# MP-Gadget/MP-Gadget

Measured on AMD Instinct MI355X. Metric: particle-updates/sec (gravity force step: PM + tree build + short-range walk), higher is better.
Workload: dtype f64; 1 GPU; 256^3 DM-only TreePM force step, Nmesh=512, s_zel ICs, all particles active, relative opening criterion (ErrTolForceAcc 0.002), TreeRcut 6, Asmth 1.5; particles=16777216, nmesh=512, parallelism=1 GPU

## Files before the change

### mp-gadget_amd/csrc/pm.h

```cpp
#pragma once
#include "../../include/mpgadget_hip.h"
#include "mpg_common.h"
#include "tree_build.h"
#include <rocfft/rocfft.h>
#include <cmath>
#include <vector>

namespace mpg {

struct FftPlan {
    rocfft_plan plan = nullptr;
    rocfft_execution_info info = nullptr;
    DevBuf<char> work;
    void create(rocfft_result_placement placement, rocfft_transform_type type, int dims, const size_t *lengths, size_t batch);
    void exec(void *in, void *out, hipStream_t st);
    void destroy();
    bool ready() const { return plan != nullptr; }
};

struct PMesh {
    double box = 0, Asmth = 0, G = 0, cellsize = 0;
    int nmesh = 0;
    bool have_plans = false;
    bool kspace_force = false;
    FftPlan plan_r2c, plan_c2r;
    DevBuf<double> real;
    DevBuf<double> rho_k;
    DevBuf<double> work_k;
    DevBuf<double> invsinc2, difffac;
    struct DepositState {
        int mode = 0, since_tune = 0;
    } dep_single, dep_slab;
    void deposit(int64_t n, const double *d_pos, const float *d_mass, const uint8_t *d_active, double *mesh, int x0, int P, DepositState &ds,
                 hipStream_t st, EventTimer *tm);
    DevBuf<unsigned long long> dep_keys_a, dep_keys_b;
    DevBuf<int> dep_idx_a, dep_idx_b;
    DevBuf<char> dep_tmp;
    bool measure_power = true, ps_valid = false;
    int ps_nmesh = 0;
    DevBuf<double> ps_acc;
    DevBuf<unsigned long long> ps_modes;
    void ps_zero(hipStream_t st);
    double asmth2() const { return pow((2 * M_PI) * Asmth / nmesh, 2); }
    double pot_factor() const { return -G / (M_PI * box); }
    enum { TR_MEASURE = 1, TR_APPLY = 2, TR_BOTH = 3 };
    template <bool XLAST, bool FUSE, bool NU> void measure_spectrum(double *rho, int ny, int y0, unsigned grid, hipStream_t st);
    template <bool XLAST, bool FUSE> void transfer_stage(int parts, double *rho, int ny, int y0, unsigned grid, hipStream_t st);
    size_t ps_lds_bytes() const { return (size_t)nmesh * 3 * sizeof(double); }

    mpg_nu_response_fn nu_fn = nullptr;
    void *nu_ctx = nullptr;
    double nu_box_mpc = 0;
    int nu_nonzero = 0;
    const char *nu_who = "gravpm_force";
    double nu_prefac = 0, nu_normfac = 1;
    DevBuf<double> nu_tab;
    DevBuf<int> nu_guess;
    double *nu_host = nullptr;
    size_t nu_host_cap = 0;
    size_t ps_lds_bytes_nu() const { return ps_lds_bytes() + (size_t)nmesh * (2 * sizeof(double) + sizeof(int)); }
    void nu_fetch(hipStream_t st, double **acc, unsigned long long **modes);
    void nu_table(const double *acc, const unsigned long long *modes, hipStream_t st);
    DepositState dep_plane;
    DevBuf<double> ps_keep;
    double plane_nu_correction(int64_t n, const double *d_pos, const float *d_mass, const uint8_t *d_active, mpg_nu_response_fn fn, void *ctx,
                               double box_mpc, hipStream_t st);
    bool hybrid_tracer = false;
    DevBuf<float> tracer_mass_buf;
    const float *tracer_mass(int64_t n, const float *d_mass, const uint8_t *d_type, hipStream_t st);

    void init(double BoxSize, double Asmth, int Nmesh, double G, hipStream_t st);
    void ensure_single();
    void destroy();
    void force(int64_t n, const double *d_pos, const float *d_mass, const uint8_t *d_active, double *d_gravpm, double *d_potential,
               hipStream_t st, EventTimer *tm);
    ~PMesh() { destroy(); }

    struct Slab {
// ... 26 lines not shown
```

### mp-gadget_amd/csrc/pm.hip

```cpp
#include "pm.h"
#include "pm_cic.h"
#include <algorithm>
#include <cmath>
#include <cstdlib>
#include <cstring>
#include <rocprim/rocprim.hpp>

namespace mpg {

#define MPG_FFT(expr)                                                                                          \
    do {                                                                                                       \
        rocfft_status _r = (expr);                                                                             \
        if(_r != rocfft_status_success)                                                                        \
            ::mpg::fail(__FILE__, __LINE__, std::string("rocFFT error ") + std::to_string((int)_r) + " in " #expr); \
    } while(0)

__global__ void __launch_bounds__(256) k_cic_deposit(int64_t n, const double *__restrict__ pos, const float *__restrict__ mass,
                                                     const uint8_t *__restrict__ active, double cellsize, int nmesh,
                                                     double *__restrict__ mesh)
{
    const int64_t i = (int64_t)blockIdx.x * blockDim.x + threadIdx.x;
    if(i >= n)
        return;
    if(active && !active[i])
        return;
    int ic[3];
    double res[3];
    cic_cell3(pos + 3 * i, cellsize, nmesh, ic, res);
    const double m = (double)mass[i];
#pragma unroll
    for(int c = 0; c < 8; c++)
        unsafeAtomicAdd(&mesh[cic_index(c, ic, nmesh)], cic_weight(c, res, 1.0) * m);
}

__global__ void __launch_bounds__(256) k_cic_deposit_slab(int64_t n, const double *__restrict__ pos, const float *__restrict__ mass,
                                                          const uint8_t *__restrict__ active, double cellsize, int nmesh, int x0, int P,
                                                          double *__restrict__ slab)
{
    const int64_t i = (int64_t)blockIdx.x * blockDim.x + threadIdx.x;
    if(i >= n)
        return;
    if(active && !active[i])
        return;
    int ic[3];
    double res[3];
    ic[0] = cic_cell(pos[3 * i], cellsize, nmesh, res[0]);
    if(!in_slab(ic[0], x0, P) && !in_slab(wrap(ic[0] + 1, nmesh), x0, P))
        return;
#pragma unroll
    for(int k = 1; k < 3; k++)
        ic[k] = cic_cell(pos[3 * i + k], cellsize, nmesh, res[k]);
    const double m = (double)mass[i];
#pragma unroll
    for(int c = 0; c < 8; c++) {
        size_t lin;
        if(cic_index_slab(c, ic, nmesh, x0, P, lin))
            unsafeAtomicAdd(&slab[lin], cic_weight(c, res, 1.0) * m);
    }
}

__global__ void __launch_bounds__(256) k_cell_keys(int64_t n, const double *__restrict__ pos, const uint8_t *__restrict__ active, double cellsize,
                                                   int nmesh, unsigned long long *__restrict__ keys, int *__restrict__ idx)
{
    const int64_t i = (int64_t)blockIdx.x * blockDim.x + threadIdx.x;
    if(i >= n)
        return;
    int ic[3];
    double res[3];
    cic_cell3(pos + 3 * i, cellsize, nmesh, ic, res);
    keys[i] = (active && !active[i]) ? ~0ull : (unsigned long long)cic_index(0, ic, nmesh);
    idx[i] = (int)i;
}

__global__ void __launch_bounds__(256) k_cic_deposit_sorted(int64_t n, const unsigned long long *__restrict__ skeys, const int *__restrict__ sidx,
                                                            const double *__restrict__ pos, const float *__restrict__ mass, double cellsize,
                                                            int nmesh, int x0, int P, double *__restrict__ mesh)
{
    const int64_t k = (int64_t)blockIdx.x * blockDim.x + threadIdx.x;
    const int lane = threadIdx.x & 63;
    unsigned long long key = ~0ull;
    double w[8];
    int ic[3] = {0, 0, 0};
#pragma unroll
    for(int c = 0; c < 8; c++)
        w[c] = 0;
    if(k < n) {
        key = skeys[k];
        if(key != ~0ull) {
            const int i = sidx[k];
            double res[3];
            cic_cell3(pos + 3 * (int64_t)i, cellsize, nmesh, ic, res);
            const double m = (double)mass[i];
#pragma unroll
            for(int c = 0; c < 8; c++)
                w[c] = cic_weight(c, res, m);
        }
    }
    const unsigned long long prev = __shfl_up(key, 1);
    bool f = lane == 0 || prev != key;
    const bool head_next = __shfl_down(f ? 1 : 0, 1) != 0;
    const bool tail = lane == 63 || head_next;
    for(int d = 1; d < 64; d <<= 1) {
        const bool f2 = __shfl_up(f ? 1 : 0, d) != 0;
        double v2[8];
#pragma unroll
        for(int c = 0; c < 8; c++)
            v2[c] = __shfl_up(w[c], d);
        if(lane >= d && !f) {
#pragma unroll
            for(int c = 0; c < 8; c++)
                w[c] += v2[c];
            f = f2;
        }
    }
    if(tail && key != ~0ull) {
#pragma unroll
        for(int c = 0; c < 8; c++) {
            size_t lin;
            if(cic_index_slab(c, ic, nmesh, x0, P, lin))
                unsafeAtomicAdd(&mesh[lin], w[c]);
        }
    }
}

__device__ __forceinline__ double sinc_unnormed(double x)
{
    if(x < 1e-5 && x > -1e-5) {
        const double x2 = x * x;
        return 1.0 - x2 / 6. + x2 * x2 / 120.;
    }
    return sin(x) / x;
}

struct FourierCell {
    int ix, iy, iz;
    long long k2;
};
template <bool XLAST>
__device__ __forceinline__ FourierCell fourier_cell(size_t ip, int nmesh, int ny, int y0)
{
    const int nz = nmesh / 2 + 1;
    FourierCell c;
    if(XLAST) {
        c.ix = (int)(ip % nmesh);
        const size_t j = ip / nmesh;
        c.iz = (int)(j % nz);
        c.iy = y0 + (int)(j / nz);
    }
    else {
        c.iz = (int)(ip % nz);
        const size_t t = ip / nz;
        c.iy = y0 + (int)(t % ny);
        c.ix = (int)(t / ny);
    }
    const int kx = c.ix <= nmesh / 2 ? c.ix : c.ix - nmesh;
    const int ky = c.iy <= nmesh / 2 ? c.iy : c.iy - nmesh;
    const int kz = c.iz;
    c.k2 = (long long)kx * kx + (long long)ky * ky + (long long)kz * kz;
    return c;
}

__device__ __forceinline__ double potential_fac(long long k2, double asmth2, double pot_factor, double f)
{
    const double smth = exp(-(double)k2 * asmth2) / (double)k2;
    return pot_factor * smth * f * f;
}

__device__ __forceinline__ int logk_bin(long long k2, double binsperunit) { return (int)floor(binsperunit * log((double)k2) / 2.); }

template <bool XLAST>
__global__ void __launch_bounds__(256) k_potential_transfer(int nmesh, int ny, int y0, double asmth2, double pot_factor,
                                                            const double *__restrict__ invsinc2, double2 *__restrict__ cplx)
{
    const int nz = nmesh / 2 + 1;
    const size_t total = (size_t)nmesh * ny * nz;
    const size_t ip = (size_t)blockIdx.x * blockDim.x + threadIdx.x;
    if(ip >= total)
        return;
    const FourierCell c = fourier_cell<XLAST>(ip, nmesh, ny, y0);
    double2 v = cplx[ip];
    if(c.k2 == 0) {
        v.x = 0.0;
        v.y = 0.0;
    }
    else {
        const double fac = potential_fac(c.k2, asmth2, pot_factor, invsinc2[c.ix] * invsinc2[c.iy] * invsinc2[c.iz]);
        v.x *= fac;
        v.y *= fac;
    }
    cplx[ip] = v;
}

struct NuArgs {
    const double *tab;
    const int *guess;
    int nonzero;
    double prefac, normfac;
    double kscale;
};

__device__ __forceinline__ double nu_factor(double x, int kint, const double *s_lk, const double *s_rt, const int *s_gs, int nonzero,
                                            double prefac)
{
    const double x0 = s_lk[0], x1 = s_lk[nonzero - 1];
    if(x < x0 && x > x0 - log(2.0))
        x = x0;
    else if(x > x1)
        x = x1;
    x = x < x0 ? x0 : x;
    int j = s_gs[kint];
    while(j > 0 && x < s_lk[j])
        j--;
    while(j < nonzero - 2 && x >= s_lk[j + 1])
        j++;
    const double x_lo = s_lk[j], x_hi = s_lk[j + 1], y_lo = s_rt[j], y_hi = s_rt[j + 1];
    return 1 + prefac * (y_lo + (x - x_lo) / (x_hi - x_lo) * (y_hi - y_lo));
}

template <bool XLAST, bool FUSE = false, bool NU = false>
__global__ void __launch_bounds__(256) k_power_spectrum(int nmesh, int ny, int y0, const double *__restrict__ invsinc2,
                                                        double2 *__restrict__ cplx, double *__restrict__ acc,
                                                        unsigned long long *__restrict__ modes, double asmth2 = 0, double pot_factor = 0,
                                                        NuArgs nu = NuArgs{})
{
    extern __shared__ double s_ps[];
    const int nbins = nmesh;
    double *s_pow = s_ps, *s_kk = s_ps + nbins;
    unsigned long long *s_n = (unsigned long long *)(s_ps + 2 * nbins);
    double *s_lk = s_ps + 3 * nbins, *s_rt = s_ps + 4 * nbins;
    int *s_gs = (int *)(s_ps + 5 * nbins);
    for(int b = threadIdx.x; b < nbins; b += blockDim.x) {
        s_pow[b] = 0;
        s_kk[b] = 0;
        s_n[b] = 0;
        if(NU) {
            s_lk[b] = nu.tab[b];
            s_rt[b] = nu.tab[nbins + b];
            s_gs[b] = nu.guess[b];
        }
    }
    __syncthreads();
    const int nz = nmesh / 2 + 1;
    const size_t total = (size_t)nmesh * ny * nz;
    const double binsperunit = (nbins - 1) / log(sqrt(3.0) * nmesh / 2.0);
    for(size_t ip = (size_t)blockIdx.x * blockDim.x + threadIdx.x; ip < total; ip += (size_t)gridDim.x * blockDim.x) {
        const FourierCell fc = fourier_cell<XLAST>(ip, nmesh, ny, y0);
        const long long k2 = fc.k2;
        double2 v = cplx[ip];
        if(k2 == 0) {
            const double m0 = v.x * v.x + v.y * v.y;
            acc[2 * nbins] = NU ? m0 * nu.normfac : m0;
            if(FUSE)
                cplx[ip] = make_double2(0.0, 0.0);
            continue;
        }
        int kint = 0;
        if(NU) {
            kint = logk_bin(k2, binsperunit);
            const double nufac = nu_factor(log(sqrt((double)k2) * nu.kscale), kint < nbins ? kint : nbins - 1, s_lk, s_rt, s_gs, nu.nonzero,
                                           nu.prefac);
            v.x *= nufac;
            v.y *= nufac;
            if(!FUSE)
                cplx[ip] = v;
        }
        const double m = v.x * v.x + v.y * v.y;
        const double f = invsinc2[fc.ix] * invsinc2[fc.iy] * invsinc2[fc.iz];
        if(FUSE) {
            const double fac = potential_fac(k2, asmth2, pot_factor, f);
            cplx[ip] = make_double2(v.x * fac, v.y * fac);
        }
        if(!NU)
            kint = logk_bin(k2, binsperunit);
        if(kint >= nbins)
            continue;
        const int w = (fc.iz == 0 || fc.iz == nmesh / 2) ? 1 : 2;
        __hip_atomic_fetch_add(&s_pow[kint], w * m * f * f, __ATOMIC_RELAXED, __HIP_MEMORY_SCOPE_WORKGROUP);
        __hip_atomic_fetch_add(&s_kk[kint], w * sqrt((double)k2), __ATOMIC_RELAXED, __HIP_MEMORY_SCOPE_WORKGROUP);
        __hip_atomic_fetch_add(&s_n[kint], (unsigned long long)w, __ATOMIC_RELAXED, __HIP_MEMORY_SCOPE_WORKGROUP);
    }
    __syncthreads();
    for(int b = threadIdx.x; b < nbins; b += blockDim.x)
        if(s_n[b]) {
            unsafeAtomicAdd(&acc[b], s_pow[b]);
            unsafeAtomicAdd(&acc[nbins + b], s_kk[b]);
            atomicAdd(&modes[b], s_n[b]);
        }
}

__global__ void __launch_bounds__(256) k_nu_correction(int nmesh, double2 *__restrict__ cplx, NuArgs nu)
{
    extern __shared__ double s_ps[];
    const int nbins = nmesh;
    double *s_lk = s_ps, *s_rt = s_ps + nbins;
    int *s_gs = (int *)(s_ps + 2 * nbins);
    for(int b = threadIdx.x; b < nbins; b += blockDim.x) {
        s_lk[b] = nu.tab[b];
        s_rt[b] = nu.tab[nbins + b];
        s_gs[b] = nu.guess[b];
    }
    __syncthreads();
    const int nz = nmesh / 2 + 1;
    const size_t total = (size_t)nmesh * nmesh * nz;
    const double binsperunit = (nbins - 1) / log(sqrt(3.0) * nmesh / 2.0);
    for(size_t ip = (size_t)blockIdx.x * blockDim.x + threadIdx.x; ip < total; ip += (size_t)gridDim.x * blockDim.x) {
        const long long k2 = fourier_cell<false>(ip, nmesh, nmesh, 0).k2;
        if(k2 == 0) {
            cplx[ip] = make_double2(0.0, 0.0);
            continue;
        }
        const int kint = logk_bin(k2, binsperunit);
        const double f = nu_factor(log(sqrt((double)k2) * nu.kscale), kint < nbins ? kint : nbins - 1, s_lk, s_rt, s_gs, nu.nonzero, nu.prefac) - 1;
        double2 v = cplx[ip];
        v.x *= f;
        v.y *= f;
        cplx[ip] = v;
    }
}

template <bool XLAST>
__global__ void __launch_bounds__(256) k_force_transfer(int nmesh, int ny, int y0, int axis, const double *__restrict__ difffac,
                                                        const double2 *__restrict__ src, double2 *__restrict__ dst, int xmul, int xoff)
{
    const int nz = nmesh / 2 + 1;
    const size_t total = (size_t)nmesh * ny * nz;
    const size_t ip = (size_t)blockIdx.x * blockDim.x + threadIdx.x;
    if(ip >= total)
        return;
    double2 v = src[ip];
    const FourierCell fc = fourier_cell<XLAST>(ip, nmesh, ny, y0);
    if(axis >= 0) {
        const double fac = difffac[axis == 0 ? fc.ix : (axis == 1 ? fc.iy : fc.iz)];
        const double t0 = -v.y * fac, t1 = v.x * fac;
        v.x = t0;
        v.y = t1;
    }
    const size_t rowsz = (size_t)ny * nz;
    if(XLAST)
        dst[ip] = v;
    else
// ... 96 lines not shown
        is2[i] = 1. / (s * s);
        const double w = k * (2 * M_PI / nmesh);
        dff[i] = -1 * (1 / 6.0 * (8 * sin(w) - sin(2 * w))) * (nmesh / box);
    }
    invsinc2.reserve(nmesh);
    difffac.reserve(nmesh);
    MPG_HIP(hipMemcpyAsync(invsinc2.p, is2.data(), nmesh * sizeof(double), hipMemcpyHostToDevice, st));
    MPG_HIP(hipMemcpyAsync(difffac.p, dff.data(), nmesh * sizeof(double), hipMemcpyHostToDevice, st));
    MPG_HIP(hipStreamSynchronize(st));
}

void FftPlan::create(rocfft_result_placement placement, rocfft_transform_type type, int dims, const size_t *lengths, size_t batch)
{
    static const bool once = (rocfft_setup(), true);
    (void)once;
    destroy();
    MPG_FFT(rocfft_plan_create(&plan, placement, type, rocfft_precision_double, (size_t)dims, lengths, batch, nullptr));
    MPG_FFT(rocfft_execution_info_create(&info));
    size_t wb = 0;
    MPG_FFT(rocfft_plan_get_work_buffer_size(plan, &wb));
    if(wb > 0) {
        work.reserve(wb + 64);
        MPG_FFT(rocfft_execution_info_set_work_buffer(info, work.p, wb));
    }
}

void FftPlan::exec(void *in, void *out, hipStream_t st)
{
    MPG_FFT(rocfft_execution_info_set_stream(info, st));
    void *ib[1] = {in}, *ob[1] = {out};
    MPG_FFT(rocfft_execute(plan, ib, out == in ? nullptr : ob, info));
}

void FftPlan::destroy()
{
    if(info)
        (void)rocfft_execution_info_destroy(info);
    if(plan)
        (void)rocfft_plan_destroy(plan);
    info = nullptr;
    plan = nullptr;
    work.release();
}

void PMesh::ensure_single()
{
    if(have_plans)
        return;
    const size_t nreal = (size_t)nmesh * nmesh * nmesh;
    const size_t ncplx = (size_t)nmesh * nmesh * (nmesh / 2 + 1);
    real.reserve(nreal);
    rho_k.reserve(2 * ncplx);
    work_k.reserve(2 * ncplx);
    const size_t len3[3] = {(size_t)nmesh, (size_t)nmesh, (size_t)nmesh};
    plan_r2c.create(rocfft_placement_notinplace, rocfft_transform_type_real_forward, 3, len3, 1);
    plan_c2r.create(rocfft_placement_notinplace, rocfft_transform_type_real_inverse, 3, len3, 1);
    have_plans = true;
}

void PMesh::ps_zero(hipStream_t st)
{
    ps_acc.reserve(2 * (size_t)nmesh + 8);
    ps_modes.reserve((size_t)nmesh + 8);
    MPG_HIP(hipMemsetAsync(ps_acc.p, 0, (2 * (size_t)nmesh + 1) * sizeof(double), st));
    MPG_HIP(hipMemsetAsync(ps_modes.p, 0, (size_t)nmesh * sizeof(unsigned long long), st));
    ps_valid = true;
    ps_nmesh = nmesh;
}

void PMesh::nu_fetch(hipStream_t st, double **acc, unsigned long long **modes)
{
    const size_t nb = (size_t)nmesh, want = 3 * nb + 1;
    if(nu_host_cap < want) {
        if(nu_host)
            (void)hipHostFree(nu_host);
        nu_host = nullptr;
        nu_host_cap = 0;
        MPG_HIP(hipHostMalloc((void **)&nu_host, want * sizeof(double), hipHostMallocDefault));
        nu_host_cap = want;
    }
    MPG_HIP(hipMemcpyAsync(nu_host, ps_acc.p, (2 * nb + 1) * sizeof(double), hipMemcpyDeviceToHost, st));
    MPG_HIP(hipMemcpyAsync(nu_host + 2 * nb + 1, ps_modes.p, nb * sizeof(unsigned long long), hipMemcpyDeviceToHost, st));
    MPG_HIP(hipStreamSynchronize(st));
    *acc = nu_host;
    *modes = (unsigned long long *)(nu_host + 2 * nb + 1);
}

void PMesh::nu_table(const double *acc, const unsigned long long *modes, hipStream_t st)
{
    const int nb = nmesh;
    MPG_CHECK(ps_lds_bytes_nu() <= 65536, std::string(nu_who) + ": the neutrino response keeps its table in LDS: Nmesh " + std::to_string(nmesh) + " is too large");
    std::vector<double> kk(nb), dcdm(nb), tab(2 * (size_t)nb, 0.0);
    std::vector<int64_t> nm(nb);
    int nonzero = 0;
    if(mpg_powerspectrum_sum(nb, acc, (const int64_t *)modes, nu_box_mpc, kk.data(), dcdm.data(), nm.data(), &nonzero) != 0)
        throw Error(mpg_last_error());
    for(int i = 0; i < nonzero; i++)
        dcdm[i] = sqrt(dcdm[i]);
    double prefac = NAN, mtot = NAN;
    double *lk = tab.data(), *rt = tab.data() + nb;
    for(int i = 0; i < nonzero; i++)
        lk[i] = rt[i] = NAN;
    const int rc = nu_fn(nu_ctx, nonzero, kk.data(), dcdm.data(), nm.data(), lk, rt, &prefac, &mtot);
    MPG_CHECK(rc == 0, std::string(nu_who) + ": the neutrino response callback failed (returned " + std::to_string(rc) + ")");
    MPG_CHECK(nonzero >= 2, std::string(nu_who) + ": neutrino response table: " + std::to_string(nonzero) + " power spectrum bins, at least 2 needed");
    MPG_CHECK(std::isfinite(prefac) && std::isfinite(mtot), std::string(nu_who) + ": neutrino response callback: nu_prefac / MtotbyMcdm not finite");
    for(int i = 0; i < nonzero; i++) {
        MPG_CHECK(std::isfinite(lk[i]) && std::isfinite(rt[i]),
                  std::string(nu_who) + ": neutrino response table: entry " + std::to_string(i) + " is not finite");
        MPG_CHECK(i == 0 || lk[i] > lk[i - 1], std::string(nu_who) + ": neutrino response table: logknu is not strictly increasing at entry " + std::to_string(i));
    }
    std::vector<int> guess(nb);
    int c = 0;
    for(int b = 0; b < nb; b++) {
        guess[b] = std::min(std::max(c - 1, 0), nonzero - 2);
        if(modes[b])
            c++;
    }
    nu_tab.reserve(2 * (size_t)nb);
    nu_guess.reserve((size_t)nb);
    memcpy(nu_host, tab.data(), 2 * (size_t)nb * sizeof(double));
    memcpy(nu_host + 2 * (size_t)nb, guess.data(), (size_t)nb * sizeof(int));
    MPG_HIP(hipMemcpyAsync(nu_tab.p, nu_host, 2 * (size_t)nb * sizeof(double), hipMemcpyHostToDevice, st));
    MPG_HIP(hipMemcpyAsync(nu_guess.p, nu_host + 2 * (size_t)nb, (size_t)nb * sizeof(int), hipMemcpyHostToDevice, st));
    nu_nonzero = nonzero;
    nu_prefac = prefac;
    nu_normfac = mtot * mtot;
    ps_zero(st);
}

__global__ void __launch_bounds__(256) k_tracer_mass(int64_t n, const float *__restrict__ mass, const uint8_t *__restrict__ type,
                                                     float *__restrict__ out)
{
    const int64_t i = (int64_t)blockIdx.x * blockDim.x + threadIdx.x;
    if(i < n)
        out[i] = type[i] == 2 ? 0.0f : mass[i];
}

const float *PMesh::tracer_mass(int64_t n, const float *d_mass, const uint8_t *d_type, hipStream_t st)
{
    if(!hybrid_tracer || n <= 0)
        return d_mass;
    MPG_CHECK(d_type != nullptr, "gravpm_force: the hybrid-neutrino deposit mask needs the particle types");
    tracer_mass_buf.reserve((size_t)n);
    hipLaunchKernelGGL(k_tracer_mass, dim3(nblk(n)), dim3(256), 0, st, n, d_mass, d_type, tracer_mass_buf.p);
    return tracer_mass_buf.p;
}

void PMesh::destroy()
{
    if(have_plans) {
        plan_r2c.destroy();
        plan_c2r.destroy();
        have_plans = false;
    }
    slab_destroy();
    real.release();
    rho_k.release();
    work_k.release();
    if(nu_host)
        (void)hipHostFree(nu_host);
    nu_host = nullptr;
    nu_host_cap = 0;
    nmesh = 0;
}

void PMesh::deposit(int64_t n, const double *d_pos, const float *d_mass, const uint8_t *d_active, double *mesh, int x0, int P, DepositState &ds,
                    hipStream_t st, EventTimer *tm)
{
    const size_t ncell = (size_t)P * nmesh * nmesh, nreal = (size_t)nmesh * nmesh * nmesh;
    const bool whole = x0 == 0 && P == nmesh;
    auto plain = [&]() {
        if(whole)
            hipLaunchKernelGGL(k_cic_deposit, dim3(nblk(n)), dim3(256), 0, st, n, d_pos, d_mass, d_active, cellsize, nmesh, mesh);
        else
            hipLaunchKernelGGL(k_cic_deposit_slab, dim3(nblk(n)), dim3(256), 0, st, n, d_pos, d_mass, d_active, cellsize, nmesh, x0, P, mesh);
    };
    auto sorted = [&]() {
        dep_keys_a.reserve((size_t)n + 1);
        dep_keys_b.reserve((size_t)n + 1);
        dep_idx_a.reserve((size_t)n + 1);
        dep_idx_b.reserve((size_t)n + 1);
        hipLaunchKernelGGL(k_cell_keys, dim3(nblk(n)), dim3(256), 0, st, n, d_pos, d_active, cellsize, nmesh, dep_keys_a.p, dep_idx_a.p);
        int bits = 1;
        while(bits < 64 && ((unsigned long long)1 << bits) < (unsigned long long)nreal)
            bits++;
        size_t tb = 0;
        MPG_HIP(rocprim::radix_sort_pairs(nullptr, tb, dep_keys_a.p, dep_keys_b.p, dep_idx_a.p, dep_idx_b.p, (size_t)n, 0, 64, st));
        dep_tmp.reserve(tb + 16);
        MPG_HIP(rocprim::radix_sort_pairs((void *)dep_tmp.p, tb, dep_keys_a.p, dep_keys_b.p, dep_idx_a.p, dep_idx_b.p, (size_t)n, 0,
                                          d_active ? 64 : bits, st));
        hipLaunchKernelGGL(k_cic_deposit_sorted, dim3(nblk(n)), dim3(256), 0, st, n, dep_keys_b.p, dep_idx_b.p, d_pos, d_mass, cellsize, nmesh, x0, P,
                           mesh);
    };
    if(const char *e = getenv("MPG_PM_DEPOSIT"))
        ds.mode = !strcmp(e, "sorted") ? 2 : 1;
    if(ds.mode == 0 || ++ds.since_tune >= 64) {
        hipEvent_t e0, e1, e2;
        MPG_HIP(hipEventCreate(&e0));
        MPG_HIP(hipEventCreate(&e1));
        MPG_HIP(hipEventCreate(&e2));
        MPG_HIP(hipEventRecord(e0, st));
        sorted();
        MPG_HIP(hipEventRecord(e1, st));
        MPG_HIP(hipMemsetAsync(mesh, 0, ncell * sizeof(double), st));
        plain();
        MPG_HIP(hipEventRecord(e2, st));
        MPG_HIP(hipEventSynchronize(e2));
        float ts = 0, tp = 0;
        MPG_HIP(hipEventElapsedTime(&ts, e0, e1));
        MPG_HIP(hipEventElapsedTime(&tp, e1, e2));
        (void)hipEventDestroy(e0);
        (void)hipEventDestroy(e1);
        (void)hipEventDestroy(e2);
        ds.mode = ts < tp ? 2 : 1;
        ds.since_tune = 0;
        if(tm)
            tm->start(st);
        MPG_HIP(hipMemsetAsync(mesh, 0, ncell * sizeof(double), st));
    }
    if(ds.mode == 2)
        sorted();
    else
        plain();
}

template <bool XLAST, bool FUSE, bool NU>
void PMesh::measure_spectrum(double *rho, int ny, int y0, unsigned grid, hipStream_t st)
{
    if(!NU)
        ps_zero(st);
    const NuArgs na = NU ? NuArgs{nu_tab.p, nu_guess.p, nu_nonzero, nu_prefac, nu_normfac, 2 * M_PI / nu_box_mpc} : NuArgs{};
    hipLaunchKernelGGL((k_power_spectrum<XLAST, FUSE, NU>), dim3(grid), dim3(256), NU ? ps_lds_bytes_nu() : ps_lds_bytes(), st, nmesh, ny, y0,
                       invsinc2.p, (double2 *)rho, ps_acc.p, ps_modes.p, FUSE ? asmth2() : 0.0, FUSE ? pot_factor() : 0.0, na);
}

template <bool XLAST, bool FUSE>
void PMesh::transfer_stage(int parts, double *rho, int ny, int y0, unsigned grid, hipStream_t st)
{
    if((parts & TR_MEASURE) && (nu_fn || (measure_power && !FUSE)))
        measure_spectrum<XLAST, false, false>(rho, ny, y0, grid, st);
    if(parts == TR_BOTH && nu_fn) {
        double *acc;
        unsigned long long *modes;
        nu_fetch(st, &acc, &modes);
        nu_table(acc, modes, st);
    }
    if(!(parts & TR_APPLY))
        return;
    if(nu_fn)
        measure_spectrum<XLAST, FUSE, true>(rho, ny, y0, grid, st);
    else if(FUSE && measure_power)
        measure_spectrum<XLAST, FUSE, false>(rho, ny, y0, grid, st);
    if(!FUSE || !(nu_fn || measure_power))
        hipLaunchKernelGGL(k_potential_transfer<XLAST>, dim3(nblk((size_t)nmesh * ny * (nmesh / 2 + 1))), dim3(256), 0, st, nmesh, ny, y0, asmth2(),
                           pot_factor(), invsinc2.p, (double2 *)rho);
}

double PMesh::plane_nu_correction(int64_t n, const double *d_pos, const float *d_mass, const uint8_t *d_active, mpg_nu_response_fn fn, void *ctx,
                                  double box_mpc, hipStream_t st)
{
    MPG_CHECK(nmesh > 0, "potential planes: the massive-neutrino correction needs the PM mesh (gravpm_init_periodic first)");
    MPG_CHECK(!slab.ready, "potential planes: the massive-neutrino correction is not available while the mesh is in its slab-decomposed form");
    MPG_CHECK(fn && box_mpc > 0, "potential planes: the massive-neutrino correction needs a callback and BoxSize_in_MPC > 0");
    ensure_single();
    const size_t nreal = (size_t)nmesh * nmesh * nmesh, nb = (size_t)nmesh;
    const bool had_ps = ps_valid && ps_nmesh == nmesh;
    if(had_ps) {
        ps_keep.reserve(3 * nb + 1);
        MPG_HIP(hipMemcpyAsync(ps_keep.p, ps_acc.p, (2 * nb + 1) * sizeof(double), hipMemcpyDeviceToDevice, st));
        MPG_HIP(hipMemcpyAsync(ps_keep.p + 2 * nb + 1, ps_modes.p, nb * sizeof(unsigned long long), hipMemcpyDeviceToDevice, st));
    }
    struct Restore {
        PMesh *pm;
        mpg_nu_response_fn fn;
        void *ctx;
        double box_mpc, prefac, normfac;
        int nonzero;
        bool had_ps;
        hipStream_t st;
        ~Restore()
        {
            pm->nu_who = "gravpm_force";
            pm->nu_fn = fn;
            pm->nu_ctx = ctx;
            pm->nu_box_mpc = box_mpc;
            pm->nu_prefac = prefac;
            pm->nu_normfac = normfac;
            pm->nu_nonzero = nonzero;
            pm->ps_valid = had_ps;
            if(had_ps) {
                const size_t nb = (size_t)pm->nmesh;
                (void)hipMemcpyAsync(pm->ps_acc.p, pm->ps_keep.p, (2 * nb + 1) * sizeof(double), hipMemcpyDeviceToDevice, st);
                (void)hipMemcpyAsync(pm->ps_modes.p, pm->ps_keep.p + 2 * nb + 1, nb * sizeof(unsigned long long), hipMemcpyDeviceToDevice, st);
            }
        }
    } restore{this, nu_fn, nu_ctx, nu_box_mpc, nu_prefac, nu_normfac, nu_nonzero, had_ps, st};
    MPG_HIP(hipMemsetAsync(real.p, 0, nreal * sizeof(double), st));
    if(n > 0)
        deposit(n, d_pos, d_mass, d_active, real.p, 0, nmesh, dep_plane, st, nullptr);
    plan_r2c.exec(real.p, rho_k.p, st);
    measure_spectrum<false, false, false>(rho_k.p, nmesh, 0, 2048, st);
    double total_mass = 0;
    MPG_HIP(hipMemcpyAsync(&total_mass, rho_k.p, sizeof(double), hipMemcpyDeviceToHost, st));
    double *acc;
    unsigned long long *modes;
    nu_fetch(st, &acc, &modes);
    MPG_CHECK(total_mass > 0, "potential planes: cannot build a potential plane from zero active particle mass");
    nu_who = "potential planes";
    nu_fn = fn;
    nu_ctx = ctx;
    nu_box_mpc = box_mpc;
    nu_table(acc, modes, st);
    const NuArgs na{nu_tab.p, nu_guess.p, nu_nonzero, nu_prefac, nu_normfac, 2 * M_PI / nu_box_mpc};
    hipLaunchKernelGGL(k_nu_correction, dim3(2048), dim3(256), (size_t)nmesh * (2 * sizeof(double) + sizeof(int)), st, nmesh, (double2 *)rho_k.p, na);
    MPG_HIP(hipGetLastError());
    plan_c2r.exec(rho_k.p, real.p, st);
    return total_mass;
}

void PMesh::force(int64_t n, const double *d_pos, const float *d_mass, const uint8_t *d_active, double *d_gravpm, double *d_potential,
                  hipStream_t st, EventTimer *tm)
{
    MPG_CHECK(nmesh > 0, "gravpm_force called before gravpm_init_periodic");
    MPG_CHECK(!slab.ready, "gravpm_force: the mesh is in its slab-decomposed form (use the pm_slab calls)");
    ensure_single();
    const size_t nreal = (size_t)nmesh * nmesh * nmesh;
    const size_t ncplx = (size_t)nmesh * nmesh * (nmesh / 2 + 1);
    float t_fft = 0, t_tr = 0, t_ro = 0;
    auto lap = [&](float &sum) {
        float t;
        if(tm) {
            tm->lap(st, &t);
            sum += t;
        }
    };
    if(tm)
        tm->start(st);
    MPG_HIP(hipMemsetAsync(real.p, 0, nreal * sizeof(double), st));
    if(n > 0)
        deposit(n, d_pos, d_mass, d_active, real.p, 0, nmesh, dep_single, st, tm);
    if(tm)
        tm->lap(st, &tm->t.pm_deposit);
    plan_r2c.exec(real.p, rho_k.p, st);
    lap(t_fft);
    static const bool fuse_ps = !(getenv("MPG_PM_FUSE_PS") && getenv("MPG_PM_FUSE_PS")[0] == '0');
    if(fuse_ps)
        transfer_stage<false, true>(TR_BOTH, rho_k.p, nmesh, 0, 2048, st);
    else
        transfer_stage<false, false>(TR_BOTH, rho_k.p, nmesh, 0, 2048, st);
    lap(t_tr);
    if(!kspace_force) {
        plan_c2r.exec(rho_k.p, real.p, st);
        lap(t_fft);
        if(n > 0)
            hipLaunchKernelGGL(k_cic_readout_stencil, dim3(nblk(n)), dim3(256), 0, st, n, d_pos, d_active, cellsize, nmesh, (double)nmesh / box,
                               (const double *)real.p, d_gravpm, d_potential);
        lap(t_ro);
    }
    else
        for(int f = 0; f < 4; f++) {
        const int axis = f - 1;
        if(f == 0 && !d_potential)
            continue;
        hipLaunchKernelGGL(k_force_transfer<false>, dim3(nblk(ncplx)), dim3(256), 0, st, nmesh, nmesh, 0, axis, difffac.p,
                           (const double2 *)rho_k.p, (double2 *)work_k.p, 1, 0);
        lap(t_tr);
        plan_c2r.exec(work_k.p, real.p, st);
        lap(t_fft);
        if(n > 0) {
            if(f == 0)
                hipLaunchKernelGGL(k_cic_readout, dim3(nblk(n)), dim3(256), 0, st, n, d_pos, d_active, cellsize, nmesh, real.p, 3, d_potential);
            else
                hipLaunchKernelGGL(k_cic_readout, dim3(nblk(n)), dim3(256), 0, st, n, d_pos, d_active, cellsize, nmesh, real.p, axis, d_gravpm);
        }
        lap(t_ro);
    }
    MPG_HIP(hipGetLastError());
    if(tm && tm->enabled) {
        tm->t.pm_fft = t_fft;
        tm->t.pm_transfer = t_tr;
        tm->t.pm_readout = t_ro;
        tm->t.pm_total = tm->t.pm_deposit + t_fft + t_tr + t_ro;
    }
}


__global__ void __launch_bounds__(256) k_slab_pack_a(int nmesh, int P, int Py, const double2 *__restrict__ C, double2 *__restrict__ sendA)
{
    const int nz = nmesh / 2 + 1;
    const size_t total = (size_t)P * nmesh * nz;
    const size_t ip = (size_t)blockIdx.x * blockDim.x + threadIdx.x;
    if(ip >= total)
        return;
    const int iz = (int)(ip % nz);
    const size_t t = ip / nz;
    const int y = (int)(t % nmesh);
    const int xl = (int)(t / nmesh);
    const int d = y / Py, yl = y - d * Py;
    sendA[(((size_t)d * P + xl) * Py + yl) * nz + iz] = C[ip];
}

__global__ void __launch_bounds__(256) k_slab_unpack_b(int nmesh, int P, int Py, const double2 *__restrict__ recvB, double2 *__restrict__ C)
{
    const int nz = nmesh / 2 + 1;
    const size_t total = (size_t)P * nmesh * nz;
// ... 11 lines not shown
__global__ void __launch_bounds__(256) k_transpose(int rows, int cols, const double2 *__restrict__ in, size_t in_ld, double2 *__restrict__ out,
                                                   size_t out_ld)
{
    __shared__ double2 tile[32][33];
    const int tx = threadIdx.x & 31, ty = threadIdx.x >> 5;
    const int c0 = blockIdx.x * 32, r0 = blockIdx.y * 32;
#pragma unroll
    for(int k = 0; k < 32; k += 8) {
        const int r = r0 + ty + k, c = c0 + tx;
        if(r < rows && c < cols)
            tile[ty + k][tx] = in[(size_t)r * in_ld + c];
    }
    __syncthreads();
#pragma unroll
    for(int k = 0; k < 32; k += 8) {
        const int c = c0 + ty + k, r = r0 + tx;
        if(r < rows && c < cols)
            out[(size_t)c * out_ld + r] = tile[tx][ty + k];
    }
}

void PMesh::slab_destroy()
{
    if(slab.ready) {
        slab.p2d_r2c.destroy();
        slab.p2d_c2r.destroy();
        slab.p1d_fwd.destroy();
        slab.p1d_inv.destroy();
        slab.ready = false;
    }
    slab.phi.release();
    slab.force.release();
    slab.C.release();
    slab.rho_k.release();
    slab.work.release();
}

void PMesh::slab_init(int rank, int world)
{
    MPG_CHECK(nmesh > 0, "pm_slab_init called before gravpm_init_periodic");
    MPG_CHECK(world >= 1 && rank >= 0 && rank < world, "pm_slab_init: bad rank / world");
    MPG_CHECK(nmesh % world == 0, "pm_slab_init: Nmesh must be a multiple of the number of GPUs");
    slab_destroy();
    slab.rank = rank;
    slab.world = world;
    slab.P = slab.Py = nmesh / world;
    const int nz = nmesh / 2 + 1;
    const size_t S = (size_t)slab.Py * nz;
    MPG_CHECK(slab.P >= 3, "pm_slab_init: at least 3 mesh planes per GPU are needed");
    slab.phi.reserve((size_t)(slab.P + 5) * nmesh * nmesh);
    slab.force.reserve((size_t)(slab.P + 1) * nmesh * nmesh);
    slab.C.reserve(2 * (size_t)slab.P * nmesh * nz);
    slab.rho_k.reserve(2 * (size_t)nmesh * S);
    if(have_plans) {
        plan_r2c.destroy();
        plan_c2r.destroy();
        have_plans = false;
    }
    real.release();
    rho_k.release();
    work_k.release();
    const size_t len2[2] = {(size_t)nmesh, (size_t)nmesh}, len1[1] = {(size_t)nmesh};
    slab.p2d_r2c.create(rocfft_placement_notinplace, rocfft_transform_type_real_forward, 2, len2, (size_t)slab.P);
    slab.p2d_c2r.create(rocfft_placement_notinplace, rocfft_transform_type_real_inverse, 2, len2, (size_t)slab.P);
    slab.p1d_fwd.create(rocfft_placement_inplace, rocfft_transform_type_complex_forward, 1, len1, S);
    slab.p1d_inv.create(rocfft_placement_inplace, rocfft_transform_type_complex_inverse, 1, len1, S);
    slab.work.reserve(2 * (size_t)nmesh * S);
    slab.ready = true;
}

void PMesh::slab_forward_a(int64_t n, const double *d_pos, const float *d_mass, double *sendA, hipStream_t st)
{
    MPG_CHECK(slab.ready, "pm_slab: not initialised");
    const int nz = nmesh / 2 + 1;
    const size_t nreal = (size_t)slab.P * nmesh * nmesh;
    MPG_HIP(hipMemsetAsync(slab.force.p, 0, nreal * sizeof(double), st));
    if(n > 0)
        deposit(n, d_pos, d_mass, nullptr, slab.force.p, slab.rank * slab.P, slab.P, dep_slab, st, nullptr);
    slab.p2d_r2c.exec(slab.force.p, slab.C.p, st);
    hipLaunchKernelGGL(k_slab_pack_a, dim3(nblk((size_t)slab.P * nmesh * nz)), dim3(256), 0, st, nmesh, slab.P, slab.Py, (const double2 *)slab.C.p,
                       (double2 *)sendA);
    MPG_HIP(hipGetLastError());
}

void PMesh::slab_forward_b(double *recvA, double *sendB, hipStream_t st)
{
    slab_forward_b1(recvA, st);
    slab_forward_b2(sendB, st);
}

void PMesh::slab_forward_b1(double *recvA, hipStream_t st)
{
    MPG_CHECK(slab.ready, "pm_slab: not initialised");
    const int nz = nmesh / 2 + 1;
    const int y0 = slab.rank * slab.Py;
    const size_t S = (size_t)slab.Py * nz;
    const dim3 tgrid_f((unsigned)((S + 31) / 32), (unsigned)((nmesh + 31) / 32));
    hipLaunchKernelGGL(k_transpose, tgrid_f, dim3(256), 0, st, nmesh, (int)S, (const double2 *)recvA, S, (double2 *)slab.rho_k.p, (size_t)nmesh);
    slab.p1d_fwd.exec(slab.rho_k.p, slab.rho_k.p, st);
    transfer_stage<true, false>(TR_MEASURE, slab.rho_k.p, slab.Py, y0, 1024, st);
}

void PMesh::slab_forward_b2(double *sendB, hipStream_t st)
{
    MPG_CHECK(slab.ready, "pm_slab: not initialised");
    const int nz = nmesh / 2 + 1;
    const int y0 = slab.rank * slab.Py;
    const size_t S = (size_t)slab.Py * nz;
    const dim3 tgrid_b((unsigned)((nmesh + 31) / 32), (unsigned)((S + 31) / 32));
    transfer_stage<true, false>(TR_APPLY, slab.rho_k.p, slab.Py, y0, 1024, st);
    slab.p1d_inv.exec(slab.rho_k.p, slab.rho_k.p, st);
// ... 55 lines not shown
```

Measured before the change: 237.4 million particles/s.

## Fuse x-axis FFT passes with PM transfer and spectrum into one kernel

Replaces the full 3D r2c/c2r rocFFT plans with batched 2D plans over the y/z axes plus a custom kernel that performs the x-axis forward FFT, applies the potential transfer function and power-spectrum binning, then runs the inverse x-axis FFT in LDS. This removes two full passes over the complex mesh, since the transfer stage and the x-direction FFT passes no longer each stream the mesh through global memory. Separately, CIC deposit now uses two threads per particle, each handling four of the eight corners. The hand-written radix-8/4/2 FFT trades rocFFT's tuning for custom code, with possible register and LDS pressure and numerical-accuracy risk.

```diff
diff --git a/mp-gadget_amd/csrc/pm.h b/mp-gadget_amd/csrc/pm.h
--- a/mp-gadget_amd/csrc/pm.h
+++ b/mp-gadget_amd/csrc/pm.h
@@ -24,6 +24,13 @@
     bool have_plans = false;
     bool kspace_force = false;
     FftPlan plan_r2c, plan_c2r;
+    FftPlan plan2_r2c, plan2_c2r;
+    DevBuf<double> xp_tw;
+    int xp_blocks = 0;
+    bool xpass_usable() const;
+    void ensure_3d();
+    void ensure_xpass(hipStream_t st);
+    void xpass_solve(hipStream_t st);
     DevBuf<double> real;
     DevBuf<double> rho_k;
     DevBuf<double> work_k;
diff --git a/mp-gadget_amd/csrc/pm.hip b/mp-gadget_amd/csrc/pm.hip
--- a/mp-gadget_amd/csrc/pm.hip
+++ b/mp-gadget_amd/csrc/pm.hip
@@ -19,7 +19,9 @@
                                                      const uint8_t *__restrict__ active, double cellsize, int nmesh,
                                                      double *__restrict__ mesh)
 {
-    const int64_t i = (int64_t)blockIdx.x * blockDim.x + threadIdx.x;
+    const int64_t t = (int64_t)blockIdx.x * blockDim.x + threadIdx.x;
+    const int64_t i = t >> 1;
+    const int h = (int)(t & 1);
     if(i >= n)
         return;
     if(active && !active[i])
@@ -29,8 +31,10 @@
     cic_cell3(pos + 3 * i, cellsize, nmesh, ic, res);
     const double m = (double)mass[i];
 #pragma unroll
-    for(int c = 0; c < 8; c++)
+    for(int q = 0; q < 4; q++) {
+        const int c = 4 * h + q;
         unsafeAtomicAdd(&mesh[cic_index(c, ic, nmesh)], cic_weight(c, res, 1.0) * m);
+    }
 }
 
 __global__ void __launch_bounds__(256) k_cic_deposit_slab(int64_t n, const double *__restrict__ pos, const float *__restrict__ mass,
@@ -136,6 +140,13 @@
     int ix, iy, iz;
     long long k2;
 };
+__device__ __forceinline__ long long fourier_k2(int ix, int iy, int iz, int nmesh)
+{
+    const int kx = ix <= nmesh / 2 ? ix : ix - nmesh;
+    const int ky = iy <= nmesh / 2 ? iy : iy - nmesh;
+    const int kz = iz;
+    return (long long)kx * kx + (long long)ky * ky + (long long)kz * kz;
+}
 template <bool XLAST>
 __device__ __forceinline__ FourierCell fourier_cell(size_t ip, int nmesh, int ny, int y0)
 {
@@ -153,10 +164,7 @@
         c.iy = y0 + (int)(t % ny);
         c.ix = (int)(t / ny);
     }
-    const int kx = c.ix <= nmesh / 2 ? c.ix : c.ix - nmesh;
-    const int ky = c.iy <= nmesh / 2 ? c.iy : c.iy - nmesh;
-    const int kz = c.iz;
-    c.k2 = (long long)kx * kx + (long long)ky * ky + (long long)kz * kz;
+    c.k2 = fourier_k2(c.ix, c.iy, c.iz, nmesh);
     return c;
 }
 
@@ -215,6 +223,62 @@
         j++;
     const double x_lo = s_lk[j], x_hi = s_lk[j + 1], y_lo = s_rt[j], y_hi = s_rt[j + 1];
     return 1 + prefac * (y_lo + (x - x_lo) / (x_hi - x_lo) * (y_hi - y_lo));
+}
+
+struct PsLds {
+    double *pow, *kk;
+    unsigned long long *n;
+    const double *lk, *rt;
+    const int *gs;
+};
+
+__device__ __forceinline__ double ps_binsperunit(int nmesh) { return (nmesh - 1) / log(sqrt(3.0) * nmesh / 2.0); }
+
+template <bool FUSE, bool NU>
+__device__ __forceinline__ bool spectrum_mode(const FourierCell &fc, int nmesh, double binsperunit, const double *__restrict__ invsinc2, double2 &v,
+                                              const PsLds &s, double *__restrict__ acc, double asmth2, double pot_factor, const NuArgs &nu)
+{
+    const int nbins = nmesh;
+    const long long k2 = fc.k2;
+    if(k2 == 0) {
+        const double m0 = v.x * v.x + v.y * v.y;
+        acc[2 * nbins] = NU ? m0 * nu.normfac : m0;
+        if(FUSE)
+            v = make_double2(0.0, 0.0);
+        return FUSE;
+    }
+    int kint = 0;
+    if(NU) {
+        kint = logk_bin(k2, binsperunit);
+        const double nufac = nu_factor(log(sqrt((double)k2) * nu.kscale), kint < nbins ? kint : nbins - 1, s.lk, s.rt, s.gs, nu.nonzero, nu.prefac);
+        v.x *= nufac;
+        v.y *= nufac;
+    }
+    const double m = v.x * v.x + v.y * v.y;
+    const double f = invsinc2[fc.ix] * invsinc2[fc.iy] * invsinc2[fc.iz];
+    if(FUSE) {
+        const double fac = potential_fac(k2, asmth2, pot_factor, f);
+        v = make_double2(v.x * fac, v.y * fac);
+    }
+    if(!NU)
+        kint = logk_bin(k2, binsperunit);
+    if(kint < nbins) {
+        const int w = (fc.iz == 0 || fc.iz == nmesh / 2) ? 1 : 2;
+        __hip_atomic_fetch_add(&s.pow[kint], w * m * f * f, __ATOMIC_RELAXED, __HIP_MEMORY_SCOPE_WORKGROUP);
+        __hip_atomic_fetch_add(&s.kk[kint], w * sqrt((double)k2), __ATOMIC_RELAXED, __HIP_MEMORY_SCOPE_WORKGROUP);
+        __hip_atomic_fetch_add(&s.n[kint], (unsigned long long)w, __ATOMIC_RELAXED, __HIP_MEMORY_SCOPE_WORKGROUP);
+    }
+    return FUSE || NU;
+}
+
+__device__ __forceinline__ void spectrum_flush(int nbins, const PsLds &s, double *__restrict__ acc, unsigned long long *__restrict__ modes)
+{
+    for(int b = threadIdx.x; b < nbins; b += blockDim.x)
+        if(s.n[b]) {
+            unsafeAtomicAdd(&acc[b], s.pow[b]);
+            unsafeAtomicAdd(&acc[nbins + b], s.kk[b]);
+            atomicAdd(&modes[b], s.n[b]);
+        }
 }
 
 template <bool XLAST, bool FUSE = false, bool NU = false>
@@ -240,52 +304,200 @@
         }
     }
     __syncthreads();
+    const PsLds s{s_pow, s_kk, s_n, s_lk, s_rt, s_gs};
     const int nz = nmesh / 2 + 1;
     const size_t total = (size_t)nmesh * ny * nz;
-    const double binsperunit = (nbins - 1) / log(sqrt(3.0) * nmesh / 2.0);
+    const double binsperunit = ps_binsperunit(nbins);
     for(size_t ip = (size_t)blockIdx.x * blockDim.x + threadIdx.x; ip < total; ip += (size_t)gridDim.x * blockDim.x) {
-        const FourierCell fc = fourier_cell<XLAST>(ip, nmesh, ny, y0);
-        const long long k2 = fc.k2;
         double2 v = cplx[ip];
-        if(k2 == 0) {
-            const double m0 = v.x * v.x + v.y * v.y;
-            acc[2 * nbins] = NU ? m0 * nu.normfac : m0;
-            if(FUSE)
-                cplx[ip] = make_double2(0.0, 0.0);
-            continue;
+        if(spectrum_mode<FUSE, NU>(fourier_cell<XLAST>(ip, nmesh, ny, y0), nmesh, binsperunit, invsinc2, v, s, acc, asmth2, pot_factor, nu))
+            cplx[ip] = v;
+    }
+    __syncthreads();
+    spectrum_flush(nbins, s, acc, modes);
+}
+
+__device__ __forceinline__ double2 xp_mul(double2 a, double2 b) { return make_double2(a.x * b.x - a.y * b.y, a.x * b.y + a.y * b.x); }
+template <int DIR> __device__ __forceinline__ double2 xp_mul_i(double2 a)
+{
+    return DIR < 0 ? make_double2(a.y, -a.x) : make_double2(-a.y, a.x);
+}
+__device__ __forceinline__ void xp_dft2(double2 &a, double2 &b)
+{
+    const double2 t = a;
+    a = make_double2(t.x + b.x, t.y + b.y);
+    b = make_double2(t.x - b.x, t.y - b.y);
+}
+template <int DIR> __device__ __forceinline__ void xp_dft4(double2 &v0, double2 &v1, double2 &v2, double2 &v3)
+{
+    xp_dft2(v0, v2);
+    xp_dft2(v1, v3);
+    v3 = xp_mul_i<DIR>(v3);
+    xp_dft2(v0, v1);
+    xp_dft2(v2, v3);
+    const double2 t = v1;
+    v1 = v2;
+    v2 = t;
+}
+template <int DIR> __device__ __forceinline__ void xp_dft8(double2 v[8], int s )
+{
+    const double h = 0.70710678118654752440;
+#pragma unroll
+    for(int n = 0; n < 4; n++)
+        xp_dft2(v[n * s], v[(n + 4) * s]);
+    {
+        const double2 a = v[5 * s], b = v[7 * s];
+        v[5 * s] = DIR < 0 ? make_double2((a.x + a.y) * h, (a.y - a.x) * h) : make_double2((a.x - a.y) * h, (a.y + a.x) * h);
+        v[6 * s] = xp_mul_i<DIR>(v[6 * s]);
+        v[7 * s] = DIR < 0 ? make_double2((b.y - b.x) * h, -(b.x + b.y) * h) : make_double2(-(b.x + b.y) * h, (b.x - b.y) * h);
+    }
+    xp_dft4<DIR>(v[0], v[1 * s], v[2 * s], v[3 * s]);
+    xp_dft4<DIR>(v[4 * s], v[5 * s], v[6 * s], v[7 * s]);
+    const double2 e1 = v[1 * s], e2 = v[2 * s], e3 = v[3 * s], o0 = v[4 * s], o1 = v[5 * s], o2 = v[6 * s];
+    v[1 * s] = o0;
+    v[2 * s] = e1;
+    v[3 * s] = o1;
+    v[4 * s] = e2;
+    v[5 * s] = o2;
+    v[6 * s] = e3;
+}
+
+template <int N> __device__ constexpr int xp_radix(int Ns)
+{
+    int n = 0;
+    for(int m = N; m > 1; m >>= 1)
+        n++;
+    return Ns == 1 && n % 3 ? 1 << (n % 3) : 8;
+}
+
+template <int N, int DIR, int Ns> __device__ __forceinline__ void xp_pass(double2 v[8], int j, const double2 *__restrict__ tw)
+{
+    constexpr int r = xp_radix<N>(Ns), nb = 8 / r;
+#pragma unroll
+    for(int u = 0; u < nb; u++) {
+        if(Ns > 1) {
+            const int k = (j + u * (N / 8)) % Ns;
+#pragma unroll
+            for(int t = 1; t < r; t++) {
+                double2 w = tw[t * k * (N / (Ns * r))];
+                if(DIR > 0)
+                    w.y = -w.y;
+                v[u + t * nb] = xp_mul(v[u + t * nb], w);
+            }
         }
-        int kint = 0;
-        if(NU) {
-            kint = logk_bin(k2, binsperunit);
-            const double nufac = nu_factor(log(sqrt((double)k2) * nu.kscale), kint < nbins ? kint : nbins - 1, s_lk, s_rt, s_gs, nu.nonzero,
-                                           nu.prefac);
-            v.x *= nufac;
-            v.y *= nufac;
-            if(!FUSE)
-                cplx[ip] = v;
+        if(r == 8)
+            xp_dft8<DIR>(v + u, nb);
+        else if(r == 4)
+            xp_dft4<DIR>(v[u], v[u + nb], v[u + 2 * nb], v[u + 3 * nb]);
+        else
+            xp_dft2(v[u], v[u + nb]);
+    }
+}
+
+template <int N, int Ns> __device__ __forceinline__ int xp_out(int j, int u, int t)
+{
+    constexpr int r = xp_radix<N>(Ns);
+    const int jb = j + u * (N / 8), k = jb % Ns;
+    return (jb - k) * r + k + t * Ns;
+}
+
+template <int N, int Ns> __device__ __forceinline__ void xp_scatter(const double2 v[8], int j, double2 *buf, int ld, int c)
+{
+    constexpr int r = xp_radix<N>(Ns), nb = 8 / r;
+#pragma unroll
+    for(int u = 0; u < nb; u++)
+#pragma unroll
+        for(int t = 0; t < r; t++)
+            buf[xp_out<N, Ns>(j, u, t) * ld + c] = v[u + t * nb];
+}
+template <int N> __device__ __forceinline__ void xp_gather(double2 v[8], int j, const double2 *buf, int ld, int c)
+{
+#pragma unroll
+    for(int q = 0; q < 8; q++)
+        v[q] = buf[(j + q * (N / 8)) * ld + c];
+}
+
+template <int N, int DIR, int Ns> __device__ __forceinline__ void xp_transform(double2 v[8], int j, int c, int ld, double2 *tile, const double2 *__restrict__ tw)
+{
+    constexpr int r = xp_radix<N>(Ns);
+    xp_pass<N, DIR, Ns>(v, j, tw);
+    if constexpr(Ns * r < N) {
+        __syncthreads();
+        xp_scatter<N, Ns>(v, j, tile, ld, c);
+        __syncthreads();
+        xp_gather<N>(v, j, tile, ld, c);
+        xp_transform<N, DIR, Ns * r>(v, j, c, ld, tile, tw);
+    }
+}
+
+constexpr int xp_cols(int N) { return N <= 512 ? 8 : 4; }
+constexpr int xp_waves(int N)
+{
+    const int lds = N * xp_cols(N) * 16 + 3 * N * 8, blocks = 2 * lds <= 160 * 1024 ? 2 : 1, w = blocks * (N / 8 * xp_cols(N)) / 256;
+    return w > 1 ? w : 1;
+}
+constexpr bool xp_supported(int N) { return N == 64 || N == 128 || N == 256 || N == 512 || N == 1024; }
+
+template <int N>
+__global__ void __launch_bounds__(N / 8 * xp_cols(N), xp_waves(N)) k_xpass_solve(const double2 *__restrict__ tw, const double *__restrict__ invsinc2,
+                                                                    double2 *__restrict__ cplx, double *__restrict__ acc,
+                                                                    unsigned long long *__restrict__ modes, double asmth2, double pot_factor)
+{
+    constexpr int TC = xp_cols(N), nz = N / 2 + 1, ntile = N / 2 / TC + 1, nbins = N;
+    extern __shared__ __attribute__((aligned(16))) double2 s_xp[];
+    double2 *tile = s_xp;
+    double *s_pow = (double *)(tile + N * TC);
+    const PsLds s{s_pow, s_pow + nbins, (unsigned long long *)(s_pow + 2 * nbins), nullptr, nullptr, nullptr};
+    for(int b = threadIdx.x; b < nbins; b += blockDim.x) {
+        s.pow[b] = 0;
+        s.kk[b] = 0;
+        s.n[b] = 0;
+    }
+    __syncthreads();
+    const int c = threadIdx.x % TC, j = threadIdx.x / TC;
+    const double bpu = ps_binsperunit(nbins);
+    const double binsperunit = __hiloint2double(__builtin_amdgcn_readfirstlane(__double2hiint(bpu)), __builtin_amdgcn_readfirstlane(__double2loint(bpu)));
+    const int items = N * ntile, per = (items + (int)gridDim.x - 1) / (int)gridDim.x;
+    const int it0 = (int)blockIdx.x * per, it1 = it0 + per < items ? it0 + per : items;
+    for(int it = it0; it < it1; it++) {
+        FourierCell fc;
+        fc.iy = it / ntile;
+        const int kz0 = (it % ntile) * TC - fc.iy % TC;
+        fc.iz = kz0 + c;
+        const bool live = fc.iz >= 0 && fc.iz < nz;
+        char *base = (char *)(cplx + ((ptrdiff_t)fc.iy * nz + kz0));
+        const unsigned off = ((unsigned)j * (N * nz) + c) * (unsigned)sizeof(double2);
+        double2 v[8];
+#pragma unroll
+        for(int q = 0; q < 8; q++)
+            v[q] = live ? *(const double2 *)(base + (size_t)q * (N / 8) * (N * nz) * sizeof(double2) + off) : make_double2(0.0, 0.0);
+        int jt = j;
+        asm volatile("" : "+v"(jt));
+        xp_transform<N, -1, 1>(v, jt, c, TC, tile, tw);
+        __syncthreads();
+#pragma unroll
+        for(int q = 0; q < 8; q++)
+            tile[(jt + q * (N / 8)) * TC + c] = v[q];
+        if(live) {
+#pragma unroll 1
+            for(int q = 0; q < 8; q++) {
+                fc.ix = jt + q * (N / 8);
+                fc.k2 = fourier_k2(fc.ix, fc.iy, fc.iz, N);
+                double2 m = tile[fc.ix * TC + c];
+                spectrum_mode<true, false>(fc, N, binsperunit, invsinc2, m, s, acc, asmth2, pot_factor, NuArgs{});
+                tile[fc.ix * TC + c] = m;
+            }
         }
-        const double m = v.x * v.x + v.y * v.y;
-        const double f = invsinc2[fc.ix] * invsinc2[fc.iy] * invsinc2[fc.iz];
-        if(FUSE) {
-            const double fac = potential_fac(k2, asmth2, pot_factor, f);
-            cplx[ip] = make_double2(v.x * fac, v.y * fac);
+        xp_gather<N>(v, jt, tile, TC, c);
+        xp_transform<N, 1, 1>(v, jt, c, TC, tile, tw);
+        if(live) {
+#pragma unroll
+            for(int q = 0; q < 8; q++)
+                *(double2 *)(base + (size_t)q * (N / 8) * (N * nz) * sizeof(double2) + off) = v[q];
         }
-        if(!NU)
-            kint = logk_bin(k2, binsperunit);
-        if(kint >= nbins)
-            continue;
-        const int w = (fc.iz == 0 || fc.iz == nmesh / 2) ? 1 : 2;
-        __hip_atomic_fetch_add(&s_pow[kint], w * m * f * f, __ATOMIC_RELAXED, __HIP_MEMORY_SCOPE_WORKGROUP);
-        __hip_atomic_fetch_add(&s_kk[kint], w * sqrt((double)k2), __ATOMIC_RELAXED, __HIP_MEMORY_SCOPE_WORKGROUP);
-        __hip_atomic_fetch_add(&s_n[kint], (unsigned long long)w, __ATOMIC_RELAXED, __HIP_MEMORY_SCOPE_WORKGROUP);
     }
     __syncthreads();
-    for(int b = threadIdx.x; b < nbins; b += blockDim.x)
-        if(s_n[b]) {
-            unsafeAtomicAdd(&acc[b], s_pow[b]);
-            unsafeAtomicAdd(&acc[nbins + b], s_kk[b]);
-            atomicAdd(&modes[b], s_n[b]);
-        }
+    spectrum_flush(nbins, s, acc, modes);
 }
 
 __global__ void __launch_bounds__(256) k_nu_correction(int nmesh, double2 *__restrict__ cplx, NuArgs nu)
@@ -488,10 +700,63 @@
     real.reserve(nreal);
     rho_k.reserve(2 * ncplx);
     work_k.reserve(2 * ncplx);
+    have_plans = true;
+}
+
+void PMesh::ensure_3d()
+{
+    if(plan_r2c.ready())
+        return;
     const size_t len3[3] = {(size_t)nmesh, (size_t)nmesh, (size_t)nmesh};
     plan_r2c.create(rocfft_placement_notinplace, rocfft_transform_type_real_forward, 3, len3, 1);
     plan_c2r.create(rocfft_placement_notinplace, rocfft_transform_type_real_inverse, 3, len3, 1);
-    have_plans = true;
+}
+
+bool PMesh::xpass_usable() const { return xp_supported(nmesh) && !kspace_force && !nu_fn && measure_power; }
+
+using XpKernel = void (*)(const double2 *, const double *, double2 *, double *, unsigned long long *, double, double);
+static XpKernel xp_kernel(int nmesh)
+{
+    switch(nmesh) {
+    case 64: return k_xpass_solve<64>;
+    case 128: return k_xpass_solve<128>;
+    case 256: return k_xpass_solve<256>;
+    case 512: return k_xpass_solve<512>;
+    case 1024: return k_xpass_solve<1024>;
+    }
+    return nullptr;
+}
+static size_t xp_lds_bytes(int nmesh) { return (size_t)nmesh * xp_cols(nmesh) * sizeof(double2) + (size_t)nmesh * 3 * sizeof(double); }
+
+void PMesh::ensure_xpass(hipStream_t st)
+{
+    if(plan2_r2c.ready())
+        return;
+    const size_t len2[2] = {(size_t)nmesh, (size_t)nmesh};
+    plan2_r2c.create(rocfft_placement_notinplace, rocfft_transform_type_real_forward, 2, len2, (size_t)nmesh);
+    plan2_c2r.create(rocfft_placement_notinplace, rocfft_transform_type_real_inverse, 2, len2, (size_t)nmesh);
+    std::vector<double> tw(2 * (size_t)nmesh);
+    for(int m = 0; m < nmesh; m++) {
+        const long double a = -2 * M_PIl * m / nmesh;
+        tw[2 * m] = (double)cosl(a);
+        tw[2 * m + 1] = (double)sinl(a);
+    }
+    xp_tw.reserve(tw.size());
+    MPG_HIP(hipMemcpyAsync(xp_tw.p, tw.data(), tw.size() * sizeof(double), hipMemcpyHostToDevice, st));
+    MPG_HIP(hipStreamSynchronize(st));
+    MPG_HIP(hipFuncSetAttribute((const void *)xp_kernel(nmesh), hipFuncAttributeMaxDynamicSharedMemorySize, (int)xp_lds_bytes(nmesh)));
+    int dev = 0, cus = 0;
+    MPG_HIP(hipGetDevice(&dev));
+    MPG_HIP(hipDeviceGetAttribute(&cus, hipDeviceAttributeMultiprocessorCount, dev));
+    const int items = nmesh * (nmesh / 2 / xp_cols(nmesh) + 1);
+    xp_blocks = std::max(1, std::min(items, 2 * cus));
+}
+
+void PMesh::xpass_solve(hipStream_t st)
+{
+    ps_zero(st);
+    hipLaunchKernelGGL(xp_kernel(nmesh), dim3(xp_blocks), dim3(nmesh / 8 * xp_cols(nmesh)), xp_lds_bytes(nmesh), st, (const double2 *)xp_tw.p,
+                       (const double *)invsinc2.p, (double2 *)rho_k.p, ps_acc.p, ps_modes.p, asmth2(), pot_factor());
 }
 
 void PMesh::ps_zero(hipStream_t st)
@@ -585,11 +850,11 @@
 
 void PMesh::destroy()
 {
-    if(have_plans) {
-        plan_r2c.destroy();
-        plan_c2r.destroy();
-        have_plans = false;
-    }
+    plan_r2c.destroy();
+    plan_c2r.destroy();
+    plan2_r2c.destroy();
+    plan2_c2r.destroy();
+    have_plans = false;
     slab_destroy();
     real.release();
     rho_k.release();
@@ -608,7 +873,7 @@
     const bool whole = x0 == 0 && P == nmesh;
     auto plain = [&]() {
         if(whole)
-            hipLaunchKernelGGL(k_cic_deposit, dim3(nblk(n)), dim3(256), 0, st, n, d_pos, d_mass, d_active, cellsize, nmesh, mesh);
+            hipLaunchKernelGGL(k_cic_deposit, dim3(nblk(2 * n)), dim3(256), 0, st, n, d_pos, d_mass, d_active, cellsize, nmesh, mesh);
         else
             hipLaunchKernelGGL(k_cic_deposit_slab, dim3(nblk(n)), dim3(256), 0, st, n, d_pos, d_mass, d_active, cellsize, nmesh, x0, P, mesh);
     };
@@ -700,6 +965,7 @@
     MPG_CHECK(!slab.ready, "potential planes: the massive-neutrino correction is not available while the mesh is in its slab-decomposed form");
     MPG_CHECK(fn && box_mpc > 0, "potential planes: the massive-neutrino correction needs a callback and BoxSize_in_MPC > 0");
     ensure_single();
+    ensure_3d();
     const size_t nreal = (size_t)nmesh * nmesh * nmesh, nb = (size_t)nmesh;
     const bool had_ps = ps_valid && ps_nmesh == nmesh;
     if(had_ps) {
@@ -778,16 +1044,30 @@
         deposit(n, d_pos, d_mass, d_active, real.p, 0, nmesh, dep_single, st, tm);
     if(tm)
         tm->lap(st, &tm->t.pm_deposit);
-    plan_r2c.exec(real.p, rho_k.p, st);
-    lap(t_fft);
     static const bool fuse_ps = !(getenv("MPG_PM_FUSE_PS") && getenv("MPG_PM_FUSE_PS")[0] == '0');
-    if(fuse_ps)
-        transfer_stage<false, true>(TR_BOTH, rho_k.p, nmesh, 0, 2048, st);
-    else
-        transfer_stage<false, false>(TR_BOTH, rho_k.p, nmesh, 0, 2048, st);
-    lap(t_tr);
+    const char *xe = getenv("MPG_PM_XPASS");
+    const bool xpass = fuse_ps && xpass_usable() && !(xe && xe[0] == '0');
+    if(xpass) {
+        ensure_xpass(st);
+        plan2_r2c.exec(real.p, rho_k.p, st);
+        lap(t_fft);
+        xpass_solve(st);
+        lap(t_tr);
+        plan2_c2r.exec(rho_k.p, real.p, st);
+    }
+    else {
+        ensure_3d();
+        plan_r2c.exec(real.p, rho_k.p, st);
+        lap(t_fft);
+        if(fuse_ps)
+            transfer_stage<false, true>(TR_BOTH, rho_k.p, nmesh, 0, 2048, st);
+        else
+            transfer_stage<false, false>(TR_BOTH, rho_k.p, nmesh, 0, 2048, st);
+        lap(t_tr);
+    }
     if(!kspace_force) {
-        plan_c2r.exec(rho_k.p, real.p, st);
+        if(!xpass)
+            plan_c2r.exec(rho_k.p, real.p, st);
         lap(t_fft);
         if(n > 0)
             hipLaunchKernelGGL(k_cic_readout_stencil, dim3(nblk(n)), dim3(256), 0, st, n, d_pos, d_active, cellsize, nmesh, (double)nmesh / box,
@@ -905,11 +1185,11 @@
     slab.force.reserve((size_t)(slab.P + 1) * nmesh * nmesh);
     slab.C.reserve(2 * (size_t)slab.P * nmesh * nz);
     slab.rho_k.reserve(2 * (size_t)nmesh * S);
-    if(have_plans) {
-        plan_r2c.destroy();
-        plan_c2r.destroy();
-        have_plans = false;
-    }
+    plan_r2c.destroy();
+    plan_c2r.destroy();
+    plan2_r2c.destroy();
+    plan2_c2r.destroy();
+    have_plans = false;
     real.release();
     rho_k.release();
     work_k.release();
```

Measured after the change: 242.8 million particles/s, median of 6. 1.02x the previous value.
